# Lindeby/toric-RL-decoder

Hardware: AMD Instinct MI355X
Metric: env steps/sec (batched) at d=7 p=0.1 (higher is better)
Workload: dtype u64

## Files before the change

### include/toricenv.h

```cpp
#ifndef TORICENV_H
#define TORICENV_H

#include <stdint.h>

#ifdef __cplusplus
extern "C" {
#endif

#define TQ_VERSION 200

#define TQ_OK 0
#define TQ_E_INVALID (-1)
#define TQ_E_HIP (-2)
#define TQ_E_CAPACITY (-3)
#define TQ_E_ACTION (-4)
#define TQ_E_INDEX (-5)
#define TQ_E_RESET (-6)

#define TQ_F32 0
#define TQ_F16 1
#define TQ_BF16 2
#define TQ_U8 3

#define TQ_PERR_FIXED 0
// ... 12 lines not shown
int tq_set_min_qubit_errors(tq_env* h, int n_errors);
int tq_set_perror_schedule(tq_env* h, int strategy, double p_start, double p_final, double p_delta);

int tq_stack_alloc(int device, uint64_t bytes, void** out);
int tq_stack_free(void* ptr);

int tq_set_xcd_bias(int bias);
int tq_get_xcd_bias(void);
int tq_env_set_xcd_bias(tq_env* h, int bias);
int tq_env_get_xcd_bias(const tq_env* h);

int tq_num_envs(const tq_env* h);
int tq_size(const tq_env* h);

int tq_reset_all(tq_env* h, const double* p_err, void* stream);
int tq_reset_idx(tq_env* h, const int32_t* idx, int n_idx, const double* p_err, void* stream);

int tq_step(tq_env* h, const int32_t* actions, float* rewards, uint8_t* terminals, void* stream);

int tq_get_state(tq_env* h, uint8_t* out, void* stream);
int tq_get_state_idx(tq_env* h, const int32_t* idx, int n_idx, uint8_t* out, void* stream);
int tq_get_qubits(tq_env* h, uint8_t* out, void* stream);
int tq_set_qubits(tq_env* h, const uint8_t* qubits, void* stream);
int tq_get_counters(tq_env* h, uint32_t* episodes, uint32_t* steps, void* stream);
int tq_eval_ground_state(tq_env* h, uint8_t* out, void* stream);
int tq_is_terminal(tq_env* h, uint8_t* out, void* stream);

int tq_persp_count(tq_env* h, int32_t* counts, int64_t* offsets, void* stream);
int tq_persp_write(tq_env* h, const int64_t* offsets, void* out, int32_t* positions,
                   int64_t capacity, int dtype, void* stream);
int tq_persp_write_range(tq_env* h, const int64_t* offsets, int first, int count, void* out,
                         int32_t* positions, int64_t capacity, int dtype, void* stream);

int tq_states_reserve(int d, int n_max);
int tq_states_persp_count(int d, int n, const uint8_t* states, int32_t* counts, int64_t* offsets,
                          void* stream);
int tq_states_persp_write(int d, int n, const uint8_t* states, const int64_t* offsets, void* out,
                          int32_t* positions, int64_t capacity, int dtype, void* stream);

int tq_select_action(tq_env* h, const float* q_table, const int64_t* offsets,
                     const int32_t* positions, const double* eps, int32_t* actions,
                     float* q_values, void* stream);

int tq_states_select_action(int n, const float* q_table, const int64_t* offsets,
                            const int32_t* positions, const double* eps, uint64_t seed,
                            uint64_t call_counter, int64_t first_id, int32_t* actions,
                            float* q_values, void* stream);

int tq_states_check(void* stream);

int tq_segment_max(const float* q_table, const int64_t* offsets, int n, const int32_t* largest,
                   float* out, void* stream);

int tq_transition_write(tq_env* h, const int32_t* actions, uint8_t* persp, uint8_t* next_persp,
                        int32_t* actions_out, void* stream);

int tq_states_transition(int d, int n, const uint8_t* states, const uint8_t* next_states,
                         const int32_t* actions, uint8_t* persp, uint8_t* next_persp,
                         int32_t* actions_out, void* stream);

int64_t tq_transition_block_bytes(int d, int64_t cap);
int tq_transition_unpack(int d, const void* block, int64_t cap, int64_t first, int64_t count,
                         uint8_t* persp, uint8_t* next_persp, int32_t* actions, float* rewards,
                         uint8_t* terminals, float* priorities, void* stream);
int tq_block_priorities(int d, void* block, int64_t cap, int n_envs, int n_steps,
                        const float* q_values, double discount, void* stream);
// ... 30 lines not shown
```

### toric-rl-decoder_amd/_lib.py

```python
import ctypes as C
import glob
import os
import subprocess

import numpy as np
import torch

_HERE = os.path.dirname(os.path.abspath(__file__))
LIB_PATH = os.path.join(_HERE, "libtoricenv.so")
CSRC = os.path.join(_HERE, "csrc")

TQ_F32, TQ_F16, TQ_BF16, TQ_U8 = 0, 1, 2, 3
TQ_PERR_FIXED, TQ_PERR_LINEAR, TQ_PERR_RANDOM = 0, 1, 2
TQ_E_INVALID, TQ_E_HIP, TQ_E_CAPACITY, TQ_E_ACTION, TQ_E_INDEX, TQ_E_RESET = -1, -2, -3, -4, -5, -6

_vp, _i, _i64, _u64, _d = C.c_void_p, C.c_int, C.c_int64, C.c_uint64, C.c_double
SYMBOLS = [
    ("tq_version", _i, []),
    ("tq_last_error", C.c_char_p, []),
    ("tq_create", _i, [C.POINTER(_vp), _i, _i, _i, _u64, _i64]),
    ("tq_destroy", _i, [_vp]),
    ("tq_set_params", _i, [_vp, _d, _d, _i]),
    ("tq_set_min_qubit_errors", _i, [_vp, _i]),
    ("tq_set_perror_schedule", _i, [_vp, _i, _d, _d, _d]),
    ("tq_stack_alloc", _i, [_i, _u64, C.POINTER(_vp)]),
    ("tq_stack_free", _i, [_vp]),
    ("tq_set_xcd_bias", _i, [_i]),
    ("tq_get_xcd_bias", _i, []),
    ("tq_env_set_xcd_bias", _i, [_vp, _i]),
    ("tq_env_get_xcd_bias", _i, [_vp]),
    ("tq_num_envs", _i, [_vp]),
    ("tq_size", _i, [_vp]),
    ("tq_reset_all", _i, [_vp, _vp, _vp]),
    ("tq_reset_idx", _i, [_vp, _vp, _i, _vp, _vp]),
    ("tq_step", _i, [_vp, _vp, _vp, _vp, _vp]),
    ("tq_get_state", _i, [_vp, _vp, _vp]),
    ("tq_get_state_idx", _i, [_vp, _vp, _i, _vp, _vp]),
    ("tq_get_qubits", _i, [_vp, _vp, _vp]),
    ("tq_set_qubits", _i, [_vp, _vp, _vp]),
    ("tq_get_counters", _i, [_vp, _vp, _vp, _vp]),
    ("tq_eval_ground_state", _i, [_vp, _vp, _vp]),
    ("tq_is_terminal", _i, [_vp, _vp, _vp]),
    ("tq_persp_count", _i, [_vp, _vp, _vp, _vp]),
    ("tq_persp_write", _i, [_vp, _vp, _vp, _vp, _i64, _i, _vp]),
    ("tq_persp_write_range", _i, [_vp, _vp, _i, _i, _vp, _vp, _i64, _i, _vp]),
    ("tq_states_reserve", _i, [_i, _i]),
    ("tq_states_persp_count", _i, [_i, _i, _vp, _vp, _vp, _vp]),
    ("tq_states_persp_write", _i, [_i, _i, _vp, _vp, _vp, _vp, _i64, _i, _vp]),
    ("tq_select_action", _i, [_vp, _vp, _vp, _vp, _vp, _vp, _vp, _vp]),
    ("tq_states_select_action", _i, [_i, _vp, _vp, _vp, _vp, _u64, _u64, _i64, _vp, _vp, _vp]),
    ("tq_states_check", _i, [_vp]),
    ("tq_segment_max", _i, [_vp, _vp, _i, _vp, _vp, _vp]),
    ("tq_transition_write", _i, [_vp, _vp, _vp, _vp, _vp, _vp]),
    ("tq_states_transition", _i, [_i, _i, _vp, _vp, _vp, _vp, _vp, _vp, _vp]),
    ("tq_transition_block_bytes", _i64, [_i, _i64]),
    ("tq_transition_unpack", _i, [_i, _vp, _i64, _i64, _i64, _vp, _vp, _vp, _vp, _vp, _vp, _vp]),
    ("tq_block_priorities", _i, [_i, _vp, _i64, _i, _i, _vp, _d, _vp]),
    ("tq_actor_step", _i, [_vp, _vp, _vp, _vp, _vp, _vp, _i64, _i64, _vp]),
    ("tq_check", _i, [_vp, _vp]),
    ("tq_replay_create", _i, [C.POINTER(_vp), _i, _i64, _d, _i, _u64, _i]),
    ("tq_replay_destroy", _i, [_vp]),
    ("tq_replay_save_block", _i, [_vp, _vp, _i64, _vp]),
    ("tq_replay_filled", _i64, [_vp, _vp]),
    ("tq_replay_sample", _i, [_vp, _i, _d, _vp, _vp, _vp, _vp, _vp, _vp, _vp, _vp, _vp, _vp, _vp]),
    ("tq_replay_get", _i, [_vp, _vp, _i, _vp, _vp, _vp, _vp, _vp, _vp, _vp]),
    ("tq_replay_update", _i, [_vp, _vp, _vp, _i, _vp]),
    ("tq_replay_reset_alpha", _i, [_vp, _d, _vp]),
    ("tq_replay_leaves", _i, [_vp, _vp, _vp]),
    ("tq_replay_tree_nodes", _i64, [_vp]),
    ("tq_replay_tree", _i, [_vp, _vp, _vp]),
    ("tq_replay_check", _i, [_vp, _vp]),
]

_lib = None


class ToricEnvError(RuntimeError):
    pass
# ... 47 lines not shown
        raise ToricEnvError("no HIP device visible to PyTorch-ROCm: the toric env has no CPU fallback")
    dev = torch.device("cuda", torch.cuda.current_device()) if device is None else torch.device(device)
    if dev.type != "cuda":
        raise ValueError(f"device must be a cuda (ROCm) device, got {dev}")
    return torch.device("cuda", dev.index if dev.index is not None else torch.cuda.current_device())


def to_device(x, dtype, device):
    if x is None:
        return None
    if not torch.is_tensor(x):
        x = torch.as_tensor(np.array(x, copy=True) if isinstance(x, np.ndarray) and not x.flags.writeable else np.ascontiguousarray(x))
    return x.to(device=device, dtype=dtype).contiguous()


class Handle:

    _h = None

    def _call(self, fn, *args):
        with torch.cuda.device(self.device):
            check(fn(self._h, *args, _stream()))

    def close(self):
        if self._h is not None and self._h.value:
            getattr(self._L, self._destroy)(self._h)
            self._h = None

    def __del__(self):
        try:
            self.close()
        except Exception:
            pass
```

### toric-rl-decoder_amd/actor.py

```python
import numpy as np
import torch

from .policy import selectActionEnvSet


class ExploreLoop:

    def __init__(self, envs, stack, positions, offsets, blocks=None, flush=8, chunks=1, overlap=True, on_flush=None, pace="host"):
        assert not envs.numpy_io, "ExploreLoop needs an EnvSet with numpy_io=False"
        n = envs.no_envs
        if offsets.dtype != torch.int64 or offsets.dim() != 2 or offsets.shape[0] < 2 or offsets.shape[1] < n + 1 or offsets.shape[1] % 2:
            raise ValueError("offsets must be an int64 tensor (rows >= 2, even row length >= no_envs + 1)")
        if n % int(chunks):
            raise ValueError("no_envs must be divisible by chunks")
        self.envs, self.stack, self.positions, self.offsets = envs, stack, positions, offsets
        self.blocks, self.flush, self.chunks, self.on_flush = blocks, int(flush), int(chunks), on_flush
        if pace not in ("host", "device"):
            raise ValueError("pace must be 'host' or 'device'")
        self.pace = pace
        self.dev = envs.device
        self.A = torch.cuda.current_stream(self.dev)
        self.B = torch.cuda.Stream(device=self.dev) if overlap else self.A
        self.overlap = self.B is not self.A
        self.scanned = [torch.cuda.Event() for _ in range(2)]
        self.written = [torch.cuda.Event() for _ in range(2)]
        self.t = 0
        if self.overlap:
            self.B.wait_stream(self.A)
        with torch.cuda.stream(self.B):
            envs.perspectiveCounts(self._row(0))
            if self.overlap:
                self.scanned[0].record(self.B)

    def _row(self, t):
        return self.offsets[t % self.offsets.shape[0]][:self.envs.no_envs + 1]

    def step(self, bracket=None):
        envs, t, k = self.envs, self.t, self.t & 1
        off = self._row(t)
        if self.overlap:
            if self.pace == "host":
                self.scanned[k].synchronize()
            else:
                self.A.wait_event(self.scanned[k])
        if bracket is not None:
            bracket[0].record(self.A)
        if self.chunks == 1:
            envs.writePerspectives(self.stack, self.positions, off)
        else:
            per = envs.no_envs // self.chunks
            for c in range(self.chunks):
                envs.writePerspectives(self.stack, self.positions, off, first=c * per, count=per)
        if bracket is not None:
            bracket[1].record(self.A)
        if self.overlap:
            self.written[k].record(self.A)
        with torch.cuda.stream(self.B):
            if self.overlap and t > 0:
                self.B.wait_event(self.written[k ^ 1])
            blk = self.blocks[(t // self.flush) % len(self.blocks)] if self.blocks else None
            envs.actorStep(None, block=blk, slot=t % self.flush, want_actions=True)
            if blk is not None and (t + 1) % self.flush == 0:
                blk.computePriorities(envs.no_envs, self.flush, None, 0.95)
                if self.on_flush is not None:
                    self.on_flush(blk)
            envs.perspectiveCounts(self._row(t + 1))
            if self.overlap:
                self.scanned[k ^ 1].record(self.B)
        self.t = t + 1

    def time_writes(self, stack, steps, skip=1):
        keep = self.stack
        self.stack = stack
        evs = [(torch.cuda.Event(enable_timing=True), torch.cuda.Event(enable_timing=True)) for _ in range(int(steps))]
        for _ in range(int(skip)):
            self.step()
        for e in evs:
            self.step(e)
        self.drain()
        torch.cuda.current_stream(self.dev).synchronize()
        self.stack = keep
        return [a.elapsed_time(b) for a, b in evs]

    def drain(self):
        if self.overlap:
            self.A.wait_stream(self.B)


def computePrioritiesParallel(A, R, Q, Qns, discount):
    if not torch.is_tensor(Q):
        A, R, Q, Qns = np.asarray(A), np.asarray(R), np.asarray(Q), np.asarray(Qns)
        q_taken = np.take_along_axis(Q, (A[:, :, -1].astype(np.int64) - 1)[:, :, None], axis=2)[:, :, 0]
# ... 25 lines not shown
```

### toric-rl-decoder_amd/csrc/abi_util.hpp

```cpp
#pragma once
#include "toricenv.h"

#include <hip/hip_runtime.h>
#include <stdarg.h>
#include <stdio.h>

#include <vector>

#include "kernels.hpp"

namespace {

thread_local char g_err[512] = "";

int fail(int code, const char* fmt, ...) {
    va_list ap;
    va_start(ap, fmt);
    vsnprintf(g_err, sizeof(g_err), fmt, ap);
    va_end(ap);
    return code;
}

#define HIPCHECK(expr)                                                                         \
    do {                                                                                       \
        hipError_t _e = (expr);                                                                \
        if (_e != hipSuccess) {                                                                \
            (void)hipGetLastError();                                                           \
            return fail(TQ_E_HIP, "%s failed: %s (%s:%d)", #expr, hipGetErrorString(_e), __FILE__, __LINE__); \
        }                                                                                      \
    } while (0)

#define KCHECK() HIPCHECK(hipGetLastError())

int bad_size(int d) { return fail(TQ_E_INVALID, "unsupported lattice size d=%d (odd 3..21)", d); }
template <class F>
int by_size(int d, F&& f) { return tq::dispatch_size(d, f, bad_size); }

inline bool aligned16(const void* p) { return (reinterpret_cast<uintptr_t>(p) & 15u) == 0; }
#define REQUIRE_ALIGNED16(p, name)                                                        \
    do {                                                                                  \
        if ((p) && !aligned16(p)) return fail(TQ_E_INVALID, "%s must be 16-byte aligned", name); \
    } while (0)

template <typename... P, typename... A>
__forceinline__ int launch(void (*kernel)(P...), dim3 grid, dim3 block, hipStream_t stream, A&&... args) {
    hipLaunchKernelGGL(kernel, grid, block, 0, stream, static_cast<P>(args)...);
    KCHECK();
    return TQ_OK;
}

constexpr int BLOCK_1D = 256;
static_assert(BLOCK_1D == tq::PART_BLOCK, "block_count_partial (kernels.hpp) sums the counts of exactly one such block");
inline dim3 grid1(int64_t n) { return dim3((unsigned)((n + BLOCK_1D - 1) / BLOCK_1D)); }
template <typename... P, typename... A>
__forceinline__ int launch_1d(void (*kernel)(P...), int64_t n, hipStream_t stream, A&&... args) {
    return launch(kernel, grid1(n), dim3(BLOCK_1D), stream, args...);
}

constexpr int MAX_DEVICES = 16;

int current_device(int* dev) {
    HIPCHECK(hipGetDevice(dev));
    if (*dev < 0 || *dev >= MAX_DEVICES) return fail(TQ_E_INVALID, "device %d out of range", *dev);
    return TQ_OK;
}

int valid_device(int device) {
    int ndev = 0;
    HIPCHECK(hipGetDeviceCount(&ndev));
    if (device < 0 || device >= ndev || device >= MAX_DEVICES)
        return fail(TQ_E_INVALID, "device %d not available (%d HIP devices)", device, ndev);
    return TQ_OK;
}

struct DeviceGuard {
    int prev = -1;
    bool switched = false;
    template <class H>
    int enter(const H* h) {
// ... 46 lines not shown
```

### toric-rl-decoder_amd/csrc/kernels.hpp

```cpp
#pragma once
#include <hip/hip_runtime.h>
#include <hip/hip_fp16.h>
#include <stdint.h>

#include "env_step.hpp"

namespace tq {

template <int W>
__device__ __forceinline__ Bits<W> load_plane(const uint64_t* __restrict__ planes, int plane, int64_t N, int64_t e) {
    Bits<W> b;
#pragma unroll
    for (int k = 0; k < W; ++k) b.w[k] = planes[((int64_t)plane * W + k) * N + e];
    return b;
}
template <int W>
__device__ __forceinline__ void store_plane(uint64_t* __restrict__ planes, int plane, int64_t N, int64_t e, const Bits<W>& b) {
#pragma unroll
    for (int k = 0; k < W; ++k) planes[((int64_t)plane * W + k) * N + e] = b.w[k];
}
template <int D>
__device__ __forceinline__ typename Lat<D>::State load_state(const uint64_t* __restrict__ planes, int64_t N, int64_t e) {
    constexpr int W = Lat<D>::W;
    typename Lat<D>::State s;
// ... 334 lines not shown
        }
        const double m = discount * qn;
        const double td = ((double)b.reward[s] + m) - qv;
        pr = (float)fabs(td);
    }
    b.priority[s] = pr;
}

constexpr int SCAN_CHUNK = 2048;

__device__ __forceinline__ int64_t wave_sum64(int64_t x) {
#pragma unroll
    for (int o = 32; o > 0; o >>= 1) x += __shfl_xor(x, o, 64);
    return x;
}

__device__ __forceinline__ void scan_load8(const int32_t* __restrict__ counts, int64_t N, int64_t i0, int (&c)[8]) {
    if (i0 + 8 <= N) {
        const int4 a = *reinterpret_cast<const int4*>(counts + i0);
        const int4 b = *reinterpret_cast<const int4*>(counts + i0 + 4);
        c[0] = a.x; c[1] = a.y; c[2] = a.z; c[3] = a.w; c[4] = b.x; c[5] = b.y; c[6] = b.z; c[7] = b.w;
    } else {
#pragma unroll
        for (int k = 0; k < 8; ++k) c[k] = i0 + k < N ? counts[i0 + k] : 0;
    }
}

__global__ __launch_bounds__(256) void k_scan_partials(const int32_t* __restrict__ counts, int64_t* __restrict__ part256,
                                                       int64_t N) {
    const int64_t e = (int64_t)blockIdx.x * PART_BLOCK + threadIdx.x;
    block_count_partial(e < N ? counts[e] : 0, part256);
}

__global__ __launch_bounds__(256) void k_scan_final(const int32_t* __restrict__ counts, const int64_t* __restrict__ partial,
                                                    int64_t* __restrict__ offsets, int32_t* __restrict__ counts_out,
                                                    int64_t N, int32_t* __restrict__ split, int LG) {
    __shared__ int64_t ws[4];
    __shared__ int64_t base_s, total_s;
    const int tid = threadIdx.x, lane = tid & 63, wave = tid >> 6;
    const int64_t i0 = (int64_t)blockIdx.x * SCAN_CHUNK + tid * 8;
    int c[8];
    scan_load8(counts, N, i0, c);
    int64_t mine = 0;
#pragma unroll
    for (int k = 0; k < 8; ++k) mine += c[k];
    int64_t inc = mine;
#pragma unroll
    for (int o = 1; o < 64; o <<= 1) {
        const int64_t t = __shfl_up(inc, o, 64);
        if (lane >= o) inc += t;
    }
    if (lane == 63) ws[wave] = inc;
    if (wave == 0) {
        int64_t b = 0;
        for (int j = lane; j < (int)blockIdx.x * (SCAN_CHUNK / PART_BLOCK); j += 64) b += partial[j];
        b = wave_sum64(b);
        if (lane == 0) base_s = b;
    }
    if (wave == 1 && split) {
        int64_t b = 0;
        const int nparts = (int)((N + PART_BLOCK - 1) / PART_BLOCK);
        for (int j = lane; j < nparts; j += 64) b += partial[j];
        b = wave_sum64(b);
        if (lane == 0) total_s = b;
    }
    __syncthreads();
    int64_t run = base_s + inc - mine;
    for (int w = 0; w < wave; ++w) run += ws[w];
    int64_t o[9];
    o[0] = run;
#pragma unroll
    for (int k = 0; k < 8; ++k) o[k + 1] = o[k] + c[k];
    if (i0 + 8 <= N) {
        longlong2* dst = reinterpret_cast<longlong2*>(offsets + i0);
#pragma unroll
        for (int k = 0; k < 4; ++k) dst[k] = make_longlong2(o[2 * k], o[2 * k + 1]);
        if (counts_out) {
            *reinterpret_cast<int4*>(counts_out + i0) = make_int4(c[0], c[1], c[2], c[3]);
            *reinterpret_cast<int4*>(counts_out + i0 + 4) = make_int4(c[4], c[5], c[6], c[7]);
        }
        if (i0 + 8 == N) offsets[N] = o[8];
    } else {
#pragma unroll
        for (int k = 0; k < 8; ++k) {
            if (i0 + k < N) {
                offsets[i0 + k] = o[k];
                if (counts_out) counts_out[i0 + k] = c[k];
                if (i0 + k + 1 == N) offsets[N] = o[k + 1];
            }
        }
    }
    if (split) {
        const int64_t total = total_s;
        const int G = 1 << LG;
        if (total == 0) {
            if (blockIdx.x == 0) for (int k = tid; k <= G; k += 256) split[k] = 0;
        } else {
            auto T = [&](int64_t k) { return (int64_t)(((uint64_t)total * (uint64_t)k) >> LG); };
            auto kfloor = [&](int64_t x) {
                int64_t k = (int64_t)((double)(x + 1) * (double)G / (double)total);
                k = k < 0 ? 0 : (k > G ? G : k);
                while (k < G && T(k + 1) <= x) ++k;
                while (k > 0 && T(k) > x) --k;
                return k;
            };
            if (blockIdx.x == 0) {
                const int64_t kz = kfloor(0);
                for (int64_t k = tid; k <= kz; k += 256) split[k] = 0;
            }
            if (o[8] > o[0]) {
                const int64_t kA = kfloor(o[0]) + 1, kB = kfloor(o[8]);
                for (int64_t k = kA; k <= kB; ++k) {
                    const int64_t t = T(k);
                    int j = 0;
#pragma unroll
                    for (int q = 1; q < 8; ++q) j += o[q] < t;
                    split[k] = (int32_t)(i0 + j + 1);
                }
            }
        }
    }
}

struct bf16_t { unsigned short u; };
typedef uint32_t u32x4 __attribute__((ext_vector_type(4)));
template <typename T> struct OutEnc;
template <> struct OutEnc<float> { static constexpr int BITS = 32; static constexpr uint32_t ONE = 0x3F800000u; };
// ... 122 lines not shown
```

### toric-rl-decoder_amd/csrc/stream_write.hpp

```cpp
#pragma once
#include "kernels.hpp"

namespace tq {

constexpr int ERR_INTERNAL = 32;
constexpr int STREAM_SLOT_WORDS = 4;
constexpr int STREAM_SPIN_LIMIT = 1 << 21;

__device__ __forceinline__ uint32_t lds_peek(const uint32_t& w) {
    return (uint32_t)__builtin_amdgcn_readfirstlane((int)__hip_atomic_load(&w, __ATOMIC_RELAXED, __HIP_MEMORY_SCOPE_WORKGROUP));
}
__device__ __forceinline__ void lds_after_peek() { __builtin_amdgcn_fence(__ATOMIC_ACQUIRE, "wavefront"); }
__device__ __forceinline__ void lds_publish(uint32_t& w, uint32_t v, int lane) {
    __builtin_amdgcn_fence(__ATOMIC_RELEASE, "wavefront");
    if (lane == 0) __hip_atomic_store(&w, v, __ATOMIC_RELAXED, __HIP_MEMORY_SCOPE_WORKGROUP);
}
__device__ __forceinline__ uint64_t readlane64(uint64_t x, int l) {
    const uint32_t lo = (uint32_t)__builtin_amdgcn_readlane((int)(uint32_t)x, l);
    const uint32_t hi = (uint32_t)__builtin_amdgcn_readlane((int)(uint32_t)(x >> 32), l);
    return ((uint64_t)hi << 32) | lo;
}

template <int D, class OrFn>
__device__ __forceinline__ void emit_at(uint32_t pos, const typename Lat<D>::B& ov, const typename Lat<D>::B& op, OrFn&& orfn) {
// ... 75 lines not shown
                                                                  const int32_t* __restrict__ split, int lg, int bias,
                                                                  unsigned int* __restrict__ slots,
                                                                  unsigned long long* __restrict__ stats = nullptr) {
    using L = Lat<D>;
    using PS = PStream<D>;
    unsigned long long t_begin = 0, t_a = 0, t_rt = 0, n_items = 0, t_first = 0;
    if (STATS) { t_begin = __builtin_readcyclecounter(); t_rt = __builtin_amdgcn_s_memrealtime(); }
    auto stats_out = [&](int wv, int ln) {
        if (STATS && ln == 0) {
            unsigned long long* o = stats + ((size_t)blockIdx.x * (NS + NPW + NP) + wv) * 4;
            o[0] = __builtin_readcyclecounter() - t_begin; o[1] = t_a;
            o[2] = (t_rt << 32) | (__builtin_amdgcn_s_memrealtime() & 0xFFFFFFFFull); o[3] = (n_items & 0xFFFFull) | (t_first << 16);
        }
    };
    using Enc = OutEnc<OutT>;
    using B = typename L::B;
    constexpr int DD = L::DD, NQ = L::NQ, W = L::W;
    constexpr int VEC = 16 / (int)sizeof(OutT);
    constexpr int EPC = 64 * VEC;
    constexpr int LE = 128 / (int)sizeof(OutT);
    constexpr int LPD = 32 / VEC;
    constexpr uint32_t RING_BITS = 32u << RB_LOG, BMASK = (1u << RB_LOG) - 1u;
    constexpr uint32_t RP = 1u << RP_LOG, PMASK = RP - 1u;
    constexpr bool WHOLE = (uint32_t)NQ * NQ + 2u * NS * CPW * EPC + 4096u < RING_BITS;
    static_assert(64u * (uint32_t)NQ + 2u * NS * CPW * EPC + 4096u < RING_BITS, "bit ring too small for this lattice size");
    static_assert((uint32_t)NQ + 512u < RP, "position ring too small");
    static_assert(QS == 1 || (uint32_t)NQ + 63u <= (uint32_t)ProdTables<D, QS>::QN, "hit queue too small");
    static_assert(QS == 1 || (uint32_t)NQ * NQ + 2u * NS * CPW * EPC + 4096u < RING_BITS, "the hit queue needs lattices that fit the ring whole");
    __shared__ StreamLds<D, NS, NP, RB_LOG, RP_LOG, NPW, QS> S;

    const int wave = __builtin_amdgcn_readfirstlane(threadIdx.x >> 6), lane = threadIdx.x & 63;

    const int RR = (1 << lg) / (int)gridDim.x;
    if (!slots || bias >= RR || (offsets[e_end] - offsets[e_begin]) * (int64_t)(NQ * sizeof(OutT)) < (int64_t)(64 << 20)) bias = 0;
    const bool take = bias > 0;
    __shared__ int slot_s[2];
    if (threadIdx.x == 0) {
        int large = !(blockIdx.x & 1), idx = (int)(blockIdx.x >> 1);
        if (take) {
            unsigned xcc;
            asm volatile("s_getreg_b32 %0, hwreg(HW_REG_XCC_ID)" : "=s"(xcc));
            large = !(xcc & 1u);
            const unsigned half = gridDim.x >> 1;
            unsigned t = atomicAdd(&slots[large], 1u);
            if (t >= half) { large ^= 1; t = atomicAdd(&slots[large], 1u); }
            idx = t < half ? (int)t : -1;
        }
        slot_s[0] = large; slot_s[1] = idx;
    }
    for (uint32_t i = threadIdx.x; i < (1u << RB_LOG) / 4; i += blockDim.x) reinterpret_cast<uint4*>(S.bits)[i] = make_uint4(0u, 0u, 0u, 0u);
    if (threadIdx.x == 0) S.abort = 0u;
    if (threadIdx.x < NP) S.pq[threadIdx.x] = 0u;
    if (threadIdx.x < NPW) S.pcons[threadIdx.x] = 0u;
    if (threadIdx.x < NS) S.cons[threadIdx.x] = 0u;
    __syncthreads();
    if (threadIdx.x == 64 * NS && take) {
        __threadfence();
        if (atomicAdd(&slots[2], 1u) == gridDim.x - 1u) { slots[0] = 0u; slots[1] = 0u; __threadfence(); slots[2] = 0u; }
    }
    if (slot_s[1] < 0) {
        if (threadIdx.x == 0) atomicOr(err, ERR_INTERNAL);
        return;
    }
    const int f_lo = slot_s[1] * 2 * RR + (slot_s[0] ? 0 : RR + bias);
    const int f_hi = f_lo + (slot_s[0] ? RR + bias : RR - bias);
    int64_t e_lo, e_hi;
    if (split) {
        e_lo = split[f_lo]; e_hi = split[f_hi];
    } else {
        __shared__ int64_t cut[2];
        if (wave < 2) {
            const int64_t e = find_cut(offsets, e_begin, e_end, wave ? f_hi : f_lo, lg, lane);
            if (lane == 0) cut[wave] = e;
        }
        __syncthreads();
        e_lo = cut[0]; e_hi = cut[1];
    }
    e_lo = e_lo < e_begin ? e_begin : (e_lo > e_end ? e_end : e_lo);
    e_hi = e_hi < e_lo ? e_lo : (e_hi > e_end ? e_end : e_hi);
    const int64_t off0 = offsets[e_begin];
    int64_t p_all = offsets[e_end] - off0;
    int64_t e_stop = e_end;
    if (p_all > capacity) {
        if (blockIdx.x == 0 && threadIdx.x == 0) atomicOr(err, ERR_CAPACITY);
        int64_t lo = e_begin, hi = e_end;
        while (lo < hi) {
            const int64_t mid = (lo + hi + 1) >> 1;
            if (offsets[mid] - off0 <= capacity) lo = mid; else hi = mid - 1;
        }
        e_stop = lo;
        p_all = offsets[e_stop] - off0;
        e_lo = e_lo < e_stop ? e_lo : e_stop;
        e_hi = e_hi < e_stop ? e_hi : e_stop;
    }
    const int64_t Q0 = offsets[e_lo] - off0, Q1 = offsets[e_hi] - off0;
    if (Q0 < 0 || Q1 < Q0 || Q1 > p_all) {
        if (threadIdx.x == 0) atomicOr(err, ERR_INTERNAL);
        return;
    }
    if (p_all == 0 && e_stop == e_end) {
// ... 343 lines not shown
```

### toric-rl-decoder_amd/csrc/toricenv.hip

```cpp
#include <stdlib.h>
#include <atomic>
#include <string.h>

#include <mutex>
#include <new>

#include "abi_util.hpp"
#include "stream_write.hpp"
#include "replay.hpp"

namespace {

struct DeviceCtx {
    std::mutex mu;
    uint16_t* lut[tq::N_SIZES] = {};
    int* err = nullptr;
    void* ws = nullptr;
    size_t ws_bytes = 0;
    int num_cus = 0;
};
constexpr int SPLIT_MAX = 256;
constexpr int SPLIT_LG = 13;
constexpr int SPLIT_ENTRIES = (1 << SPLIT_LG) + 1;
constexpr int N_SLOT_SETS = 8;
// ... 41 lines not shown
        HIPCHECK(hipMalloc((void**)&c.err, sizeof(int)));
        HIPCHECK(hipMemset(c.err, 0, sizeof(int)));
    }
    if (!c.num_cus) {
        hipDeviceProp_t prop;
        HIPCHECK(hipGetDeviceProperties(&prop, dev));
        c.num_cus = prop.multiProcessorCount;
    }
    *out = c.lut[slot];
    return TQ_OK;
}

int launch_scan(const int32_t* counts, int64_t* partial, bool partial_valid, int64_t* offsets, int32_t* counts_out,
                int64_t n, hipStream_t stream, int32_t* split) {
    const unsigned blocks = (unsigned)((n + tq::SCAN_CHUNK - 1) / tq::SCAN_CHUNK);
    if (!partial_valid)
        hipLaunchKernelGGL(tq::k_scan_partials, grid1(n), dim3(BLOCK_1D), 0, stream, counts, partial, n);
    hipLaunchKernelGGL(tq::k_scan_final, dim3(blocks), dim3(256), 0, stream, counts, partial, offsets, counts_out, n, split,
                       SPLIT_LG);
    KCHECK();
    return TQ_OK;
}

template <int D, int ES>
struct StreamCfg {
    static constexpr int NS = D <= 5 ? (D == 5 && ES == 2 ? 3 : 2) : 4;
    static constexpr int NPW = (ES < 4 && D >= 5) ? 2 : 1;
    static constexpr int NP = D >= 17 ? 3 : (D >= 13 ? 8 - NPW : 16 - NS - NPW);
    static constexpr int CPW = 8, RB = 14, RP = 12;
};
template <int D, typename OutT>
int launch_persp_write_t(const uint64_t* vp, int64_t n, const int64_t* offsets, void* out, int32_t* pos,
                         int64_t capacity, int* err, hipStream_t stream, int64_t first, int64_t count,
                         const int32_t* split, unsigned int* slots, int bias) {
    using C = StreamCfg<D, (int)sizeof(OutT)>;
    if ((double)count * (2.0 * D * D) * (2.0 * D * D) / SPLIT_MAX * 1.5 > 2.0e9)
        return fail(TQ_E_INVALID, "lattice range too large for one stack write (%lld lattices of d=%d)", (long long)count, D);
    return launch(tq::k_persp_stream<D, OutT, C::NS, C::NP, C::CPW, C::RB, C::RP, false, C::NPW>, dim3(SPLIT_MAX),
                  dim3(64 * (C::NS + C::NPW + C::NP)), stream, vp, n, offsets, out, pos, capacity, err, first, first + count, split,
                  SPLIT_LG, (D >= 7 && sizeof(OutT) >= 2) ? bias : 0, slots, nullptr);
}

template <int D>
int launch_persp_write(const uint64_t* vp, int64_t n, const int64_t* offsets, void* out, int32_t* pos,
                       int64_t capacity, int dtype, int* err, hipStream_t stream, int64_t first, int64_t count,
                       const int32_t* split, unsigned int* slots = nullptr, int bias = 0) {
    if (count == 0) return TQ_OK;
    switch (dtype) {
        case TQ_F32: return launch_persp_write_t<D, float>(vp, n, offsets, out, pos, capacity, err, stream, first, count, split, slots, bias);
        case TQ_F16: return launch_persp_write_t<D, __half>(vp, n, offsets, out, pos, capacity, err, stream, first, count, split, slots, bias);
        case TQ_BF16: return launch_persp_write_t<D, tq::bf16_t>(vp, n, offsets, out, pos, capacity, err, stream, first, count, split, slots, bias);
        case TQ_U8: return launch_persp_write_t<D, uint8_t>(vp, n, offsets, out, pos, capacity, err, stream, first, count, split, slots, bias);
        default: return fail(TQ_E_INVALID, "unknown dtype %d", dtype);
    }
}

}

struct tq_env {
    int n, d, w, device;
    uint64_t seed;
    int64_t first_env;
    double terminal_reward = 100.0;
    int max_steps = 75;
    int min_err;
    tq::PerrSchedule sched = {TQ_PERR_FIXED, 0.1, 0.1, 0.1, 0.0};
    uint64_t* planes;
    uint64_t* planes_alt;
    uint64_t* prev;
    uint32_t* episodes;
    uint32_t* steps;
    int32_t* counts;
    int64_t* partial;
    bool partial_valid;
    double* p_roof;
    int* err;
    uint32_t* mark;
    uint32_t reset_epoch;
    void* tblock;
    const uint16_t* lut;
    int num_cus;
    int32_t* split[2];
    const int64_t* split_for[2];
    int split_last;
    unsigned int* slots;
// ... 194 lines not shown

int tq_get_counters(tq_env* h, uint32_t* episodes, uint32_t* steps, void* stream_) {
    HANDLE(h);
    if (episodes) HIPCHECK(hipMemcpyAsync(episodes, h->episodes, 4 * (size_t)h->n, hipMemcpyDeviceToDevice, stream));
    if (steps) HIPCHECK(hipMemcpyAsync(steps, h->steps, 4 * (size_t)h->n, hipMemcpyDeviceToDevice, stream));
    return TQ_OK;
}

int tq_eval_ground_state(tq_env* h, uint8_t* out, void* stream_) {
    HANDLE(h);
    if (!out) return fail(TQ_E_INVALID, "out is NULL");
    return by_size(h->d, [&](auto D) { return launch_1d(tq::k_flags<D()>, h->n, stream, h->planes, h->n, out, nullptr); });
}

int tq_is_terminal(tq_env* h, uint8_t* out, void* stream_) {
    HANDLE(h);
    if (!out) return fail(TQ_E_INVALID, "out is NULL");
    return by_size(h->d, [&](auto D) { return launch_1d(tq::k_flags<D()>, h->n, stream, h->planes, h->n, nullptr, out); });
}

int tq_persp_count(tq_env* h, int32_t* counts, int64_t* offsets, void* stream_) {
    HANDLE(h);
    if (!offsets) return fail(TQ_E_INVALID, "offsets is NULL");
    REQUIRE_ALIGNED16(offsets, "offsets");
    REQUIRE_ALIGNED16(counts, "counts");
    const int k = h->split_last ^ 1;
    if (int rc = launch_scan(h->counts, h->partial, h->partial_valid, offsets, counts, h->n, stream, h->split[k])) return rc;
    h->partial_valid = true;
    h->split_for[k] = offsets;
    h->split_last = k;
    return TQ_OK;
}

int tq_persp_write_range(tq_env* h, const int64_t* offsets, int first, int count, void* out, int32_t* positions,
                         int64_t capacity, int dtype, void* stream_) {
    HANDLE(h);
    if (!offsets || !out) return fail(TQ_E_INVALID, "offsets / out is NULL");
    if (capacity < 0) return fail(TQ_E_INVALID, "negative capacity");
    if (first < 0 || count < 0 || (int64_t)first + count > h->n) return fail(TQ_E_INVALID, "lattice range outside [0, n_envs)");
    REQUIRE_ALIGNED16(out, "out");
    REQUIRE_ALIGNED16(positions, "positions");
    const uint64_t* vp = h->planes + (size_t)tq::PL_V * h->w * h->n;
    const int32_t* split = nullptr;
    if (first == 0 && count == h->n) {
        if (offsets == h->split_for[h->split_last]) split = h->split[h->split_last];
        else if (offsets == h->split_for[h->split_last ^ 1]) split = h->split[h->split_last ^ 1];
    }
    unsigned int* slots = h->slots + tq::STREAM_SLOT_WORDS * (h->write_seq++ % N_SLOT_SETS);
    return by_size(h->d, [&](auto D) {
        return launch_persp_write<D()>(vp, h->n, offsets, out, positions, capacity, dtype, h->err, stream, first, count, split,
                                       slots, h->xcd_bias >= 0 ? h->xcd_bias : xcd_bias());
    });
}

int tq_persp_write(tq_env* h, const int64_t* offsets, void* out, int32_t* positions, int64_t capacity,
                   int dtype, void* stream_) {
    if (!h) return fail(TQ_E_INVALID, "NULL handle");
    return tq_persp_write_range(h, offsets, 0, h->n, out, positions, capacity, dtype, stream_);
}

static int stateless_enter(int d, hipStream_t stream, int* dev, const uint16_t** lut) {
    if (int rc = current_device(dev)) return rc;
    return get_lut(*dev, d, stream, lut);
}

struct StatesScratch {
    size_t counts_at, partial_at, bytes;
    StatesScratch(int d, int64_t n) {
        const size_t w = (size_t)(d * d + 63) / 64;
        counts_at = 2 * w * (size_t)n * 8;
        partial_at = counts_at + (((size_t)n * 4 + 32 + 15) & ~(size_t)15);
        bytes = partial_at + (((size_t)n + tq::PART_BLOCK - 1) / tq::PART_BLOCK) * 8;
    }
};

int tq_states_reserve(int d, int n_max) {
    if (!tq::size_ok(d)) return bad_size(d);
    if (n_max <= 0) return fail(TQ_E_INVALID, "n_max must be > 0");
    int dev;
    const uint16_t* lut;
    if (int rc = stateless_enter(d, nullptr, &dev, &lut)) return rc;
    DeviceCtx& c = g_ctx[dev];
    std::lock_guard<std::mutex> lock(c.mu);
    const size_t need = StatesScratch(d, n_max).bytes;
    if (c.ws_bytes < need) {
        HIPCHECK(hipDeviceSynchronize());
        if (c.ws) HIPCHECK(hipFree(c.ws));
        c.ws = nullptr; c.ws_bytes = 0;
        HIPCHECK(hipMalloc(&c.ws, need));
        HIPCHECK(hipMemset(c.ws, 0, need));
        c.ws_bytes = need;
// ... 186 lines not shown
```

### toric-rl-decoder_amd/envset.py

```python
import ctypes as C

import numpy as np
import torch

from . import _lib, stackbuf
from ._lib import TQ_BF16, TQ_F16, TQ_F32, TQ_U8, Handle, _ptr, _stream, check, require_gpu, to_device
from .stackbuf import alloc_chunked, alloc_stack, configured_xcd_bias, set_xcd_bias
from .transition import TransitionBlock, generateTransitionParallel, to_structured, transition_dtype, transition_outputs

_DTYPES = {torch.float32: TQ_F32, torch.float16: TQ_F16, torch.bfloat16: TQ_BF16, torch.uint8: TQ_U8}
_STRATEGY = {None: 0, "fixed": 0, "linear": 1, "random": 2}
SUPPORTED_SIZES = (3, 5, 7, 9, 11, 13, 15, 17, 19, 21)


class _ActionSpace:

    def __init__(self, d):
        self.low = np.array([0, 0, 0, 1])
        self.high = np.array([1, d - 1, d - 1, 3])


class ToricEnv:

    def __init__(self, config=None, device=None, seed=0):
# ... 164 lines not shown
        self._call(self._L.tq_get_qubits, _ptr(q))
        return self._out(q, np.int64)

    def setQubits(self, qubits):
        q = to_device(qubits, torch.uint8, self.device)
        if q.numel() != self.no_envs * 2 * self.size * self.size:
            raise ValueError("qubits must be (no_envs, 2, d, d)")
        self._call(self._L.tq_set_qubits, _ptr(q))

    def getCounters(self):
        ep = torch.empty(self.no_envs, dtype=torch.int32, device=self.device)
        st = torch.empty(self.no_envs, dtype=torch.int32, device=self.device)
        self._call(self._L.tq_get_counters, _ptr(ep), _ptr(st))
        return self._out(ep), self._out(st)

    def evalGroundState(self):
        out = torch.empty(self.no_envs, dtype=torch.uint8, device=self.device)
        self._call(self._L.tq_eval_ground_state, _ptr(out))
        return self._out(out, bool)

    def isTerminal(self):
        out = torch.empty(self.no_envs, dtype=torch.uint8, device=self.device)
        self._call(self._L.tq_is_terminal, _ptr(out))
        return self._out(out, bool)

    def perspectiveCounts(self, offsets=None):
        if offsets is not None:
            if offsets.dtype != torch.int64 or offsets.numel() != self.no_envs + 1 or not offsets.is_contiguous():
                raise ValueError("offsets must be a contiguous int64 tensor of no_envs + 1 elements")
            self._offsets = offsets
        self._call(self._L.tq_persp_count, _ptr(self._counts), _ptr(self._offsets))
        return self._counts, self._offsets

    def writePerspectives(self, out, positions=None, offsets=None, first=0, count=None):
        if out.dtype not in _DTYPES or not out.is_contiguous():
            raise ValueError("out must be a contiguous float32/float16/bfloat16/uint8 tensor")
        nq = 2 * self.size * self.size
        cap = out.numel() // nq
        if positions is not None and (positions.dtype != torch.int32 or positions.numel() < 3 * cap):
            raise ValueError("positions must be int32 with at least 3*capacity elements")
        off = self._offsets if offsets is None else offsets
        if first == 0 and count is None:
            self._call(self._L.tq_persp_write, _ptr(off), _ptr(out), _ptr(positions), cap, _DTYPES[out.dtype])
        else:
            count = self.no_envs - int(first) if count is None else int(count)
            self._call(self._L.tq_persp_write_range, _ptr(off), int(first), count, _ptr(out), _ptr(positions), cap,
                       _DTYPES[out.dtype])
        self._positions = positions

    def pickStackBuffer(self, candidates=4, dtype=torch.float32, capacity=None, positions=None, launches=10,
                        kinds=("torch", "chunked"), park=False, timer=None, passes=2, among=None):
        d, nq = self.size, 2 * self.size * self.size
        cap = self.no_envs * nq if capacity is None else int(capacity)
        if positions is None:
            positions = torch.empty((cap, 3), dtype=torch.int32, device=self.device)
        shape, passes = (cap, 2, d, d), max(1, int(passes))
        per_pass = max(1, int(launches) // passes)
        if among is not None:
            keep, used, room = list(among), [stackbuf.REPROBED] * len(among), 0
        else:
            keep, used = [], []
            with torch.cuda.device(self.device):
                free = torch.cuda.mem_get_info()[0]
            room, fit = stackbuf.candidates_that_fit(free, cap * nq * torch.empty((), dtype=dtype).element_size(), candidates)
            stackbuf.allocate_candidates(keep, used, fit, kinds, shape, dtype, self.device)
        if timer is None:
            timer = stackbuf.default_timer(self, positions)
        torch.cuda.synchronize(self.device)
        samples = stackbuf.time_candidates(timer, keep, passes, per_pass)
        first, more = len(keep), stackbuf.candidates_to_add(stackbuf.medians(samples), room, among is not None)
        if more:
            stackbuf.allocate_candidates(keep, used, more, kinds, shape, dtype, self.device)
            torch.cuda.synchronize(self.device)
            samples += stackbuf.time_candidates(timer, keep[first:], passes, per_pass)
        self.check()
        best = keep[stackbuf.verdict(samples)[2]]
        if park:
            self._parked = [x for x in self._parked if all(x is not y for y in keep)] + [x for x in keep if x is not best]
# ... 129 lines not shown
```

Before: 227.0 million.

## Signal write-completion events from the kernel launch and validate split table

Records the cross-stream completion event directly in the perspective-write kernel launch via hipExtLaunchKernelGGL instead of a separate event record. Stream B in the actor then waits on this native event. The scan kernel also stores the total and N in the split header, so the write kernel uses the split table only when it matches the current range and otherwise falls back to computing its own cut. This aims to cut per-step event-record overhead in the overlapped actor loop, at the cost of a new event API and a ban on use with stream capture.

```diff
diff --git a/include/toricenv.h b/include/toricenv.h
--- a/include/toricenv.h
+++ b/include/toricenv.h
@@ -68,6 +68,15 @@
 int tq_persp_write_range(tq_env* h, const int64_t* offsets, int first, int count, void* out,
                          int32_t* positions, int64_t capacity, int dtype, void* stream);
 
+typedef struct tq_event tq_event;
+int tq_event_create(tq_event** out, int device);
+int tq_event_destroy(tq_event* ev);
+int tq_persp_write_signal(tq_env* h, const int64_t* offsets, void* out, int32_t* positions,
+                          int64_t capacity, int dtype, tq_event* done, void* stream);
+int tq_persp_write_range_signal(tq_env* h, const int64_t* offsets, int first, int count, void* out,
+                                int32_t* positions, int64_t capacity, int dtype, tq_event* done, void* stream);
+int tq_stream_wait_event(tq_event* ev, void* stream);
+
 int tq_states_reserve(int d, int n_max);
 int tq_states_persp_count(int d, int n, const uint8_t* states, int32_t* counts, int64_t* offsets,
                           void* stream);
diff --git a/toric-rl-decoder_amd/_lib.py b/toric-rl-decoder_amd/_lib.py
--- a/toric-rl-decoder_amd/_lib.py
+++ b/toric-rl-decoder_amd/_lib.py
@@ -44,6 +44,11 @@
     ("tq_persp_count", _i, [_vp, _vp, _vp, _vp]),
     ("tq_persp_write", _i, [_vp, _vp, _vp, _vp, _i64, _i, _vp]),
     ("tq_persp_write_range", _i, [_vp, _vp, _i, _i, _vp, _vp, _i64, _i, _vp]),
+    ("tq_event_create", _i, [C.POINTER(_vp), _i]),
+    ("tq_event_destroy", _i, [_vp]),
+    ("tq_persp_write_signal", _i, [_vp, _vp, _vp, _vp, _i64, _i, _vp, _vp]),
+    ("tq_persp_write_range_signal", _i, [_vp, _vp, _i, _i, _vp, _vp, _i64, _i, _vp, _vp]),
+    ("tq_stream_wait_event", _i, [_vp, _vp]),
     ("tq_states_reserve", _i, [_i, _i]),
     ("tq_states_persp_count", _i, [_i, _i, _vp, _vp, _vp, _vp]),
     ("tq_states_persp_write", _i, [_i, _i, _vp, _vp, _vp, _vp, _i64, _i, _vp]),
@@ -157,3 +162,27 @@
             self.close()
         except Exception:
             pass
+
+
+class WriteEvent:
+
+    def __init__(self, device):
+        self.device = require_gpu(device)
+        self._L = load()
+        self._h = C.c_void_p(None)
+        check(self._L.tq_event_create(C.byref(self._h), self.device.index))
+
+    def wait(self, stream=None):
+        s = _stream() if stream is None else C.c_void_p(stream.cuda_stream)
+        check(self._L.tq_stream_wait_event(self._h, s))
+
+    def close(self):
+        if self._h is not None and self._h.value:
+            self._L.tq_event_destroy(self._h)
+            self._h = None
+
+    def __del__(self):
+        try:
+            self.close()
+        except Exception:
+            pass
diff --git a/toric-rl-decoder_amd/actor.py b/toric-rl-decoder_amd/actor.py
--- a/toric-rl-decoder_amd/actor.py
+++ b/toric-rl-decoder_amd/actor.py
@@ -1,6 +1,7 @@
 import numpy as np
 import torch
 
+from ._lib import WriteEvent
 from .policy import selectActionEnvSet
 
 
@@ -23,7 +24,7 @@
         self.B = torch.cuda.Stream(device=self.dev) if overlap else self.A
         self.overlap = self.B is not self.A
         self.scanned = [torch.cuda.Event() for _ in range(2)]
-        self.written = [torch.cuda.Event() for _ in range(2)]
+        self.written = [WriteEvent(self.dev) for _ in range(2)] if self.overlap else [None, None]
         self.t = 0
         if self.overlap:
             self.B.wait_stream(self.A)
@@ -45,19 +46,19 @@
                 self.A.wait_event(self.scanned[k])
         if bracket is not None:
             bracket[0].record(self.A)
+        done = self.written[k]
         if self.chunks == 1:
-            envs.writePerspectives(self.stack, self.positions, off)
+            envs.writePerspectives(self.stack, self.positions, off, done=done)
         else:
             per = envs.no_envs // self.chunks
             for c in range(self.chunks):
-                envs.writePerspectives(self.stack, self.positions, off, first=c * per, count=per)
+                envs.writePerspectives(self.stack, self.positions, off, first=c * per, count=per,
+                                       done=done if c == self.chunks - 1 else None)
         if bracket is not None:
             bracket[1].record(self.A)
-        if self.overlap:
-            self.written[k].record(self.A)
         with torch.cuda.stream(self.B):
             if self.overlap and t > 0:
-                self.B.wait_event(self.written[k ^ 1])
+                self.written[k ^ 1].wait(self.B)
             blk = self.blocks[(t // self.flush) % len(self.blocks)] if self.blocks else None
             envs.actorStep(None, block=blk, slot=t % self.flush, want_actions=True)
             if blk is not None and (t + 1) % self.flush == 0:
diff --git a/toric-rl-decoder_amd/csrc/abi_util.hpp b/toric-rl-decoder_amd/csrc/abi_util.hpp
--- a/toric-rl-decoder_amd/csrc/abi_util.hpp
+++ b/toric-rl-decoder_amd/csrc/abi_util.hpp
@@ -2,6 +2,7 @@
 #include "toricenv.h"
 
 #include <hip/hip_runtime.h>
+#include <hip/hip_ext.h>
 #include <stdarg.h>
 #include <stdio.h>
 
@@ -45,6 +46,13 @@
 template <typename... P, typename... A>
 __forceinline__ int launch(void (*kernel)(P...), dim3 grid, dim3 block, hipStream_t stream, A&&... args) {
     hipLaunchKernelGGL(kernel, grid, block, 0, stream, static_cast<P>(args)...);
+    KCHECK();
+    return TQ_OK;
+}
+template <typename... P, typename... A>
+__forceinline__ int launch_signal(void (*kernel)(P...), dim3 grid, dim3 block, hipStream_t stream, hipEvent_t done, A&&... args) {
+    if (!done) return launch(kernel, grid, block, stream, args...);
+    hipExtLaunchKernelGGL(kernel, grid, block, 0, stream, nullptr, done, 0, static_cast<P>(args)...);
     KCHECK();
     return TQ_OK;
 }
diff --git a/toric-rl-decoder_amd/csrc/kernels.hpp b/toric-rl-decoder_amd/csrc/kernels.hpp
--- a/toric-rl-decoder_amd/csrc/kernels.hpp
+++ b/toric-rl-decoder_amd/csrc/kernels.hpp
@@ -390,6 +390,7 @@
     block_count_partial(e < N ? counts[e] : 0, part256);
 }
 
+constexpr int SPLIT_HEADER = 3;
 __global__ __launch_bounds__(256) void k_scan_final(const int32_t* __restrict__ counts, const int64_t* __restrict__ partial,
                                                     int64_t* __restrict__ offsets, int32_t* __restrict__ counts_out,
                                                     int64_t N, int32_t* __restrict__ split, int LG) {
@@ -451,6 +452,9 @@
     if (split) {
         const int64_t total = total_s;
         const int G = 1 << LG;
+        if (blockIdx.x == 0 && tid == 0) {
+            split[G + 1] = (int32_t)(uint32_t)total; split[G + 2] = (int32_t)(uint32_t)((uint64_t)total >> 32); split[G + 3] = (int32_t)N;
+        }
         if (total == 0) {
             if (blockIdx.x == 0) for (int k = tid; k <= G; k += 256) split[k] = 0;
         } else {
diff --git a/toric-rl-decoder_amd/csrc/stream_write.hpp b/toric-rl-decoder_amd/csrc/stream_write.hpp
--- a/toric-rl-decoder_amd/csrc/stream_write.hpp
+++ b/toric-rl-decoder_amd/csrc/stream_write.hpp
@@ -131,7 +131,8 @@
     const int wave = __builtin_amdgcn_readfirstlane(threadIdx.x >> 6), lane = threadIdx.x & 63;
 
     const int RR = (1 << lg) / (int)gridDim.x;
-    if (!slots || bias >= RR || (offsets[e_end] - offsets[e_begin]) * (int64_t)(NQ * sizeof(OutT)) < (int64_t)(64 << 20)) bias = 0;
+    const int64_t p_tab = offsets[e_end] - offsets[e_begin];
+    if (!slots || bias >= RR || p_tab * (int64_t)(NQ * sizeof(OutT)) < (int64_t)(64 << 20)) bias = 0;
     const bool take = bias > 0;
     __shared__ int slot_s[2];
     if (threadIdx.x == 0) {
@@ -163,8 +164,14 @@
     }
     const int f_lo = slot_s[1] * 2 * RR + (slot_s[0] ? 0 : RR + bias);
     const int f_hi = f_lo + (slot_s[0] ? RR + bias : RR - bias);
+    bool by_tab = false;
+    if (split) {
+        const int G = 1 << lg;
+        const int64_t t_all = (int64_t)(((uint64_t)(uint32_t)split[G + 2] << 32) | (uint32_t)split[G + 1]);
+        by_tab = t_all == p_tab && e_begin == 0 && (int64_t)split[G + 3] == e_end;
+    }
     int64_t e_lo, e_hi;
-    if (split) {
+    if (by_tab) {
         e_lo = split[f_lo]; e_hi = split[f_hi];
     } else {
         __shared__ int64_t cut[2];
diff --git a/toric-rl-decoder_amd/csrc/toricenv.hip b/toric-rl-decoder_amd/csrc/toricenv.hip
--- a/toric-rl-decoder_amd/csrc/toricenv.hip
+++ b/toric-rl-decoder_amd/csrc/toricenv.hip
@@ -97,25 +97,28 @@
 template <int D, typename OutT>
 int launch_persp_write_t(const uint64_t* vp, int64_t n, const int64_t* offsets, void* out, int32_t* pos,
                          int64_t capacity, int* err, hipStream_t stream, int64_t first, int64_t count,
-                         const int32_t* split, unsigned int* slots, int bias) {
+                         const int32_t* split, unsigned int* slots, int bias, hipEvent_t done) {
     using C = StreamCfg<D, (int)sizeof(OutT)>;
     if ((double)count * (2.0 * D * D) * (2.0 * D * D) / SPLIT_MAX * 1.5 > 2.0e9)
         return fail(TQ_E_INVALID, "lattice range too large for one stack write (%lld lattices of d=%d)", (long long)count, D);
-    return launch(tq::k_persp_stream<D, OutT, C::NS, C::NP, C::CPW, C::RB, C::RP, false, C::NPW>, dim3(SPLIT_MAX),
-                  dim3(64 * (C::NS + C::NPW + C::NP)), stream, vp, n, offsets, out, pos, capacity, err, first, first + count, split,
-                  SPLIT_LG, (D >= 7 && sizeof(OutT) >= 2) ? bias : 0, slots, nullptr);
+    return launch_signal(tq::k_persp_stream<D, OutT, C::NS, C::NP, C::CPW, C::RB, C::RP, false, C::NPW>, dim3(SPLIT_MAX),
+                         dim3(64 * (C::NS + C::NPW + C::NP)), stream, done, vp, n, offsets, out, pos, capacity, err, first,
+                         first + count, split, SPLIT_LG, (D >= 7 && sizeof(OutT) >= 2) ? bias : 0, slots, nullptr);
 }
 
 template <int D>
 int launch_persp_write(const uint64_t* vp, int64_t n, const int64_t* offsets, void* out, int32_t* pos,
                        int64_t capacity, int dtype, int* err, hipStream_t stream, int64_t first, int64_t count,
-                       const int32_t* split, unsigned int* slots = nullptr, int bias = 0) {
-    if (count == 0) return TQ_OK;
+                       const int32_t* split, unsigned int* slots = nullptr, int bias = 0, hipEvent_t done = nullptr) {
+    if (count == 0) {
+        if (done) HIPCHECK(hipEventRecord(done, stream));
+        return TQ_OK;
+    }
     switch (dtype) {
-        case TQ_F32: return launch_persp_write_t<D, float>(vp, n, offsets, out, pos, capacity, err, stream, first, count, split, slots, bias);
-        case TQ_F16: return launch_persp_write_t<D, __half>(vp, n, offsets, out, pos, capacity, err, stream, first, count, split, slots, bias);
-        case TQ_BF16: return launch_persp_write_t<D, tq::bf16_t>(vp, n, offsets, out, pos, capacity, err, stream, first, count, split, slots, bias);
-        case TQ_U8: return launch_persp_write_t<D, uint8_t>(vp, n, offsets, out, pos, capacity, err, stream, first, count, split, slots, bias);
+        case TQ_F32: return launch_persp_write_t<D, float>(vp, n, offsets, out, pos, capacity, err, stream, first, count, split, slots, bias, done);
+        case TQ_F16: return launch_persp_write_t<D, __half>(vp, n, offsets, out, pos, capacity, err, stream, first, count, split, slots, bias, done);
+        case TQ_BF16: return launch_persp_write_t<D, tq::bf16_t>(vp, n, offsets, out, pos, capacity, err, stream, first, count, split, slots, bias, done);
+        case TQ_U8: return launch_persp_write_t<D, uint8_t>(vp, n, offsets, out, pos, capacity, err, stream, first, count, split, slots, bias, done);
         default: return fail(TQ_E_INVALID, "unknown dtype %d", dtype);
     }
 }
@@ -376,14 +379,56 @@
     return TQ_OK;
 }
 
-int tq_persp_write_range(tq_env* h, const int64_t* offsets, int first, int count, void* out, int32_t* positions,
-                         int64_t capacity, int dtype, void* stream_) {
+struct tq_event {
+    int device;
+    hipEvent_t ev;
+};
+
+int tq_event_create(tq_event** out, int device) {
+    if (!out) return fail(TQ_E_INVALID, "out is NULL");
+    *out = nullptr;
+    if (int rc = valid_device(device)) return rc;
+    DeviceGuard guard;
+    if (int rc = guard.enter_device(device)) return rc;
+    hipEvent_t ev;
+    HIPCHECK(hipEventCreateWithFlags(&ev, hipEventDisableTiming));
+    tq_event* e = new (std::nothrow) tq_event{device, ev};
+    if (!e) { (void)hipEventDestroy(ev); return fail(TQ_E_INVALID, "out of host memory"); }
+    *out = e;
+    return TQ_OK;
+}
+
+int tq_event_destroy(tq_event* ev) {
+    if (!ev) return TQ_OK;
+    DeviceGuard guard;
+    (void)guard.enter_device(ev->device);
+    (void)hipEventDestroy(ev->ev);
+    delete ev;
+    return TQ_OK;
+}
+
+int tq_stream_wait_event(tq_event* ev, void* stream_) {
+    DeviceGuard guard;
+    if (int rc = guard.enter(ev)) return rc;
+    HIPCHECK(hipStreamWaitEvent((hipStream_t)stream_, ev->ev, 0));
+    return TQ_OK;
+}
+
+int tq_persp_write_range_signal(tq_env* h, const int64_t* offsets, int first, int count, void* out, int32_t* positions,
+                                int64_t capacity, int dtype, tq_event* done, void* stream_) {
     HANDLE(h);
     if (!offsets || !out) return fail(TQ_E_INVALID, "offsets / out is NULL");
     if (capacity < 0) return fail(TQ_E_INVALID, "negative capacity");
     if (first < 0 || count < 0 || (int64_t)first + count > h->n) return fail(TQ_E_INVALID, "lattice range outside [0, n_envs)");
     REQUIRE_ALIGNED16(out, "out");
     REQUIRE_ALIGNED16(positions, "positions");
+    if (done) {
+        if (done->device != h->device) return fail(TQ_E_INVALID, "the event belongs to device %d, the handle to %d", done->device, h->device);
+        hipStreamCaptureStatus cap = hipStreamCaptureStatusNone;
+        HIPCHECK(hipStreamIsCapturing(stream, &cap));
+        if (cap != hipStreamCaptureStatusNone)
+            return fail(TQ_E_INVALID, "tq_persp_write_signal on a capturing stream: capture the plain tq_persp_write");
+    }
     const uint64_t* vp = h->planes + (size_t)tq::PL_V * h->w * h->n;
     const int32_t* split = nullptr;
     if (first == 0 && count == h->n) {
@@ -393,14 +438,25 @@
     unsigned int* slots = h->slots + tq::STREAM_SLOT_WORDS * (h->write_seq++ % N_SLOT_SETS);
     return by_size(h->d, [&](auto D) {
         return launch_persp_write<D()>(vp, h->n, offsets, out, positions, capacity, dtype, h->err, stream, first, count, split,
-                                       slots, h->xcd_bias >= 0 ? h->xcd_bias : xcd_bias());
+                                       slots, h->xcd_bias >= 0 ? h->xcd_bias : xcd_bias(), done ? done->ev : nullptr);
     });
+}
+
+int tq_persp_write_range(tq_env* h, const int64_t* offsets, int first, int count, void* out, int32_t* positions,
+                         int64_t capacity, int dtype, void* stream_) {
+    return tq_persp_write_range_signal(h, offsets, first, count, out, positions, capacity, dtype, nullptr, stream_);
+}
+
+int tq_persp_write_signal(tq_env* h, const int64_t* offsets, void* out, int32_t* positions, int64_t capacity,
+                          int dtype, tq_event* done, void* stream_) {
+    if (!h) return fail(TQ_E_INVALID, "NULL handle");
+    return tq_persp_write_range_signal(h, offsets, 0, h->n, out, positions, capacity, dtype, done, stream_);
 }
 
 int tq_persp_write(tq_env* h, const int64_t* offsets, void* out, int32_t* positions, int64_t capacity,
                    int dtype, void* stream_) {
     if (!h) return fail(TQ_E_INVALID, "NULL handle");
-    return tq_persp_write_range(h, offsets, 0, h->n, out, positions, capacity, dtype, stream_);
+    return tq_persp_write_range_signal(h, offsets, 0, h->n, out, positions, capacity, dtype, nullptr, stream_);
 }
 
 static int stateless_enter(int d, hipStream_t stream, int* dev, const uint16_t** lut) {
diff --git a/toric-rl-decoder_amd/envset.py b/toric-rl-decoder_amd/envset.py
--- a/toric-rl-decoder_amd/envset.py
+++ b/toric-rl-decoder_amd/envset.py
@@ -220,7 +220,7 @@
         self._call(self._L.tq_persp_count, _ptr(self._counts), _ptr(self._offsets))
         return self._counts, self._offsets
 
-    def writePerspectives(self, out, positions=None, offsets=None, first=0, count=None):
+    def writePerspectives(self, out, positions=None, offsets=None, first=0, count=None, done=None):
         if out.dtype not in _DTYPES or not out.is_contiguous():
             raise ValueError("out must be a contiguous float32/float16/bfloat16/uint8 tensor")
         nq = 2 * self.size * self.size
@@ -228,10 +228,14 @@
         if positions is not None and (positions.dtype != torch.int32 or positions.numel() < 3 * cap):
             raise ValueError("positions must be int32 with at least 3*capacity elements")
         off = self._offsets if offsets is None else offsets
-        if first == 0 and count is None:
+        whole = first == 0 and count is None
+        count = self.no_envs - int(first) if count is None else int(count)
+        if done is not None:
+            self._call(self._L.tq_persp_write_range_signal, _ptr(off), int(first), count, _ptr(out), _ptr(positions), cap,
+                       _DTYPES[out.dtype], done._h)
+        elif whole:
             self._call(self._L.tq_persp_write, _ptr(off), _ptr(out), _ptr(positions), cap, _DTYPES[out.dtype])
         else:
-            count = self.no_envs - int(first) if count is None else int(count)
             self._call(self._L.tq_persp_write_range, _ptr(off), int(first), count, _ptr(out), _ptr(positions), cap,
                        _DTYPES[out.dtype])
         self._positions = positions
```

After: 229.6 million, median of 6. +1.1%, better.
